# jyoung3131/oncilla

Hardware: AMD Instinct MI355X
Metric: remote put/get GiB/s + p50 ocm_alloc latency, 4 KiB-1 GiB, 1/2/4/8 MI355X (higher is better)
Workload: dtype uint8

## Files before the change

### csrc/include/ocm/xfer.h

```cpp
#pragma once
#include <hip/hip_runtime_api.h>

#include <cstdint>

#include "ocm/list.h"

namespace ocm {

struct XferArgs {
    char *lin;
    char *ext[kXferMaxExtents];
    uint64_t rem_off;
    uint64_t len;
    uint32_t unit_shift;
    uint32_t n_ext;
    uint32_t tile_shift;
    uint32_t put;
};

enum XferVariant : int {
    XFER_AUTO = 0,
    XFER_REG = 1,
    XFER_LDS = 2,
    XFER_DMA = 3,
    XFER_PCIE = 4,
    XFER_PUSH = 5,
};

struct XferTuning {
    int variant = XFER_AUTO;
    int max_blocks = 0;
    bool nontemporal = true;
    bool write_through = false;
};

struct XferDone {
    unsigned long long *flag = nullptr;
    unsigned int *cnt = nullptr;
    unsigned long long val = 0;
};

__host__ __device__ inline uint64_t xfer_first_tile(uint64_t rem_off, uint32_t tile_shift) {
    return rem_off & ~((1ull << tile_shift) - 1);
}
__host__ __device__ inline uint64_t xfer_tile_count(uint64_t rem_off, uint64_t len, uint32_t tile_shift) {
    const uint64_t mask = (1ull << tile_shift) - 1;
    return (((rem_off + len + mask) & ~mask) - (rem_off & ~mask)) >> tile_shift;
}

hipError_t xfer_normalize(XferArgs &a);

hipError_t xfer_launch(const XferArgs &a, const XferTuning &t, hipStream_t stream, const XferDone *done = nullptr);

hipError_t xfer_push_launch(const XferArgs &a, uint32_t ext_mask, int max_blocks, hipStream_t stream);

hipError_t xfer_copy(void *dst, const void *src, uint64_t bytes, const XferTuning &t, hipStream_t stream);

XferTuning xfer_tuning_from_env();

struct XferBatchOp {
    uint64_t lin_off;
    uint64_t rem_off;
    uint64_t len;
    uint64_t first_tile;
    uint32_t put;
    uint32_t pad;
};
static_assert(sizeof(XferBatchOp) == 40, "batch op layout");

constexpr int kXferInlineOps = 48;

struct XferBatchArgs : ListArgs<XferBatchOp, kXferInlineOps> {
    uint32_t abs_lin;
};
static_assert(list_args_fit<XferBatchArgs>, "kernarg segment limit");

inline uint64_t xfer_batch_plan(XferBatchOp *ops, uint32_t n, uint32_t tile_shift) {
    return list_plan(ops, n, [tile_shift](const XferBatchOp &op) {
        return op.len ? xfer_tile_count(op.rem_off, op.len, tile_shift) : 0;
    });
}
uint32_t xfer_batch_grid(uint64_t total_tiles, bool host_tier = false);
uint32_t xfer_batch_tile_shift(uint32_t n_ext, uint32_t unit_shift);
hipError_t xfer_batch_launch(const XferBatchArgs &a, const XferTuning &t, hipStream_t stream);
hipError_t xfer_batch_graph_node(hipGraph_t graph, hipGraphNode_t dep, const XferBatchArgs &a, const XferTuning &t,
// ... 119 lines not shown
```

### csrc/src/kernels/xfer.hip

```cpp
#include <hip/hip_runtime.h>

#include <cstring>

#include "ocm/xfer.h"
#include "xfer_copy.h"
#include "xfer_host.h"

namespace ocm {

namespace {

constexpr int kWaveSlice = (1 << kTileShift) / kWaves;
constexpr int kChunksPerWave = kWaveSlice / 1024;

template <class Cfg, bool MASKED = false>
__device__ __forceinline__ void copy_tiles(const XferArgs &a, uint32_t ext_mask = 0) {
    const uint64_t first = xfer_first_tile(a.rem_off, a.tile_shift);
    const uint64_t ntiles = xfer_tile_count(a.rem_off, a.len, a.tile_shift);
    const uint64_t r0 = a.rem_off;
    for (uint64_t ti = blockIdx.x; ti < ntiles; ti += gridDim.x) {
        if (MASKED && a.n_ext > 1) {
            const uint64_t lo = first + (ti << a.tile_shift);
            const uint64_t ts = lo > r0 ? lo : r0;
            const uint32_t e = (uint32_t)(ts >> a.unit_shift) % a.n_ext;
            if (!((ext_mask >> e) & 1u)) continue;
        }
        TileSpan s = tile_span(a, ti, first);
        copy_span<Cfg>(s.dst, s.src, s.n);
    }
}

template <int ST>
__global__ __launch_bounds__(kThreads) void xfer_reg_kernel(XferArgs a, XferDone d) {
    copy_tiles<BlockCopy<ST>>(a);
// ... 54 lines not shown
        }
        if (nt >= ntiles) break;
        ti = nt;
        cur = nxt;
        cur_staged = nxt_staged;
        slot ^= 1;
    }
}

template <bool NT>
__global__ __launch_bounds__(kThreads) void xfer_lds_kernel(XferArgs a, XferDone d) {
    __shared__ __attribute__((aligned(16))) char lds[2 * (1 << kTileShift)];
    const int wave = threadIdx.x >> 6, lane = threadIdx.x & 63;
    const uint64_t first = xfer_first_tile(a.rem_off, a.tile_shift);
    const uint64_t ntiles = xfer_tile_count(a.rem_off, a.len, a.tile_shift);
    uint64_t ti = blockIdx.x;
    if (ti < ntiles) lds_stream<NT>(a, lds, wave, lane, ti, first, ntiles);
    xfer_publish(d);
}

constexpr int kPcieUnroll = 2;
constexpr uint32_t kPcieTileShift = 13;
constexpr unsigned kPcieBlocksDefault = 128;

template <int SA>
using PcieCopy = CopyCfg<kThreads, kPcieUnroll, BufferAccess<kAuxNT, SA>>;

template <int SA>
__global__ __launch_bounds__(kThreads) void xfer_pcie_kernel(XferArgs a, XferDone d) {
    copy_tiles<PcieCopy<SA>>(a);
    xfer_publish(d);
}

__global__ __launch_bounds__(kThreads) void xfer_push_kernel(XferArgs a, uint32_t mask) {
    copy_tiles<BlockCopy<ST_NT>, true>(a, mask);
}

}

XferTuning xfer_tuning_from_env() {
    XferTuning t;
    const char *v = std::getenv("OCM_XFER_VARIANT");
    if (v && (!std::strcmp(v, "lds") || !std::strcmp(v, "2"))) t.variant = XFER_LDS;
    if (v && (!std::strcmp(v, "reg") || !std::strcmp(v, "1"))) t.variant = XFER_REG;
    if (v && (!std::strcmp(v, "pcie") || !std::strcmp(v, "4"))) t.variant = XFER_PCIE;
    if (v && (!std::strcmp(v, "push") || !std::strcmp(v, "5"))) t.variant = XFER_PUSH;
    t.max_blocks = kernels::env_int("OCM_XFER_BLOCKS", 0);
    t.nontemporal = kernels::env_int("OCM_XFER_NT", 1) != 0;
    t.write_through = kernels::env_int("OCM_XFER_NT", 1) == 2;
    return t;
}

hipError_t xfer_normalize(XferArgs &a) {
    if (a.n_ext < 1 || a.n_ext > (uint32_t)kXferMaxExtents) return hipErrorInvalidValue;
    a.tile_shift = kTileShift;
    if (a.n_ext > 1) {
        if (a.unit_shift < 4) return hipErrorInvalidValue;
        if (a.unit_shift < kTileShift) a.tile_shift = a.unit_shift;
    }
    return hipSuccess;
}

hipError_t xfer_launch(const XferArgs &in, const XferTuning &t, hipStream_t stream, const XferDone *done) {
    if (in.len == 0) return hipSuccess;
    XferArgs a = in;
    if (xfer_normalize(a) != hipSuccess) return hipErrorInvalidValue;
    const uint64_t ntiles = xfer_tile_count(a.rem_off, a.len, a.tile_shift);
    int variant = t.variant;
    if (variant == XFER_AUTO) variant = XFER_REG;
    const XferDone d0 = done ? *done : XferDone{};
    if (variant == XFER_PCIE) {
        if (a.tile_shift > kPcieTileShift) a.tile_shift = kPcieTileShift;
        const uint64_t tiles = xfer_tile_count(a.rem_off, a.len, a.tile_shift);
        const uint64_t cap = t.max_blocks > 0 ? (uint64_t)t.max_blocks : (uint64_t)kPcieBlocksDefault;
        const unsigned g = (unsigned)(tiles < cap ? tiles : cap);
        if (a.put && t.nontemporal)
            hipLaunchKernelGGL(xfer_pcie_kernel<kAuxSC1>, dim3(g), dim3(kThreads), 0, stream, a, d0);
        else
            hipLaunchKernelGGL(xfer_pcie_kernel<0>, dim3(g), dim3(kThreads), 0, stream, a, d0);
        return hipGetLastError();
    }
    if (a.tile_shift != kTileShift) variant = XFER_REG;
    int cap = t.max_blocks > 0 ? t.max_blocks : kernels::num_cus() * (variant == XFER_LDS ? 4 : 2);
    const unsigned grid = (unsigned)(ntiles < (uint64_t)cap ? ntiles : (uint64_t)cap);
    if (variant == XFER_LDS) {
        if (t.nontemporal)
            hipLaunchKernelGGL(xfer_lds_kernel<true>, dim3(grid), dim3(kThreads), 0, stream, a, d0);
        else
            hipLaunchKernelGGL(xfer_lds_kernel<false>, dim3(grid), dim3(kThreads), 0, stream, a, d0);
    } else {
        if (t.write_through)
            hipLaunchKernelGGL(xfer_reg_kernel<ST_WT>, dim3(grid), dim3(kThreads), 0, stream, a, d0);
        else if (t.nontemporal)
            hipLaunchKernelGGL(xfer_reg_kernel<ST_NT>, dim3(grid), dim3(kThreads), 0, stream, a, d0);
        else
            hipLaunchKernelGGL(xfer_reg_kernel<ST_PLAIN>, dim3(grid), dim3(kThreads), 0, stream, a, d0);
    }
    return hipGetLastError();
}

hipError_t xfer_push_launch(const XferArgs &in, uint32_t ext_mask, int max_blocks, hipStream_t stream) {
    if (in.len == 0 || ext_mask == 0) return hipSuccess;
    XferArgs a = in;
    if (a.put || xfer_normalize(a) != hipSuccess) return hipErrorInvalidValue;
    const uint64_t tiles = xfer_tile_count(a.rem_off, a.len, a.tile_shift);
    const uint32_t mine = (uint32_t)__builtin_popcount(ext_mask & ((1u << a.n_ext) - 1));
    const uint64_t own = a.n_ext > 1 ? (tiles * mine + a.n_ext - 1) / a.n_ext : tiles;
    const uint64_t cap = max_blocks > 0 ? (uint64_t)max_blocks : (uint64_t)kernels::num_cus() * 2;
    const unsigned g = (unsigned)(own < cap ? (own ? own : 1) : cap);
    hipLaunchKernelGGL(xfer_push_kernel, dim3(g), dim3(kThreads), 0, stream, a, ext_mask);
    return hipGetLastError();
}

hipError_t xfer_copy(void *dst, const void *src, uint64_t bytes, const XferTuning &t, hipStream_t stream) {
    XferArgs a;
// ... 12 lines not shown
```

### csrc/src/lib/config.cpp

```cpp
#include "config.h"

#include <algorithm>
#include <climits>
#include <cstdlib>
#include <cstring>

namespace ocmlib {

int env_int(const char *k, int dflt) {
    const char *v = std::getenv(k);
    return (v && *v) ? std::atoi(v) : dflt;
}

static uint64_t env_u64(const char *k, uint64_t dflt) {
    const char *v = std::getenv(k);
    return (v && *v) ? std::strtoull(v, nullptr, 0) : dflt;
}

static int env_clamped(const char *k, int dflt, int lo, int hi = INT_MAX) {
    return std::max(lo, std::min(env_int(k, dflt), hi));
}

static bool env_bool(const char *k, bool dflt) { return env_int(k, dflt ? 1 : 0) != 0; }

static uint64_t env_scaled(const char *k, uint64_t dflt, uint64_t per, int lo) {
    return per * (uint64_t)env_clamped(k, (int)(dflt / per), lo);
}

Config config_from_env() {
    Config c;
    c.rpc_timeout_ms = env_int("OCM_RPC_TIMEOUT_MS", c.rpc_timeout_ms);
    c.rpc_spin_ns = env_scaled("OCM_RPC_SPIN_US", c.rpc_spin_ns, 1000, 0);
    c.connect_timeout_ms = env_int("OCM_CONNECT_TIMEOUT_MS", c.connect_timeout_ms);
    c.shm_link = env_bool("OCM_SHM_LINK", c.shm_link);
    c.no_gpu = std::getenv("OCM_NO_GPU") != nullptr;
    c.net_streams = env_clamped("OCM_NET_STREAMS", c.net_streams, 1, 64);
    c.net_split_min = std::max<uint64_t>(4096, env_u64("OCM_NET_SPLIT_MIN", c.net_split_min));
    c.sync_mode = env_int("OCM_SYNC_MODE", c.sync_mode);
    c.n_lanes = env_int("OCM_ASYNC_LANES", c.n_lanes);
    c.pinned_keep = env_u64("OCM_PINNED_KEEP", c.pinned_keep);
    c.dev_cache_cap = env_u64("OCM_LOCAL_CACHE", c.dev_cache_cap);
    const char *he = std::getenv("OCM_HOST_ENGINE");
    c.host_engine_kernel = !(he && !std::strcmp(he, "sdma"));
    c.host_kernel_max = env_u64("OCM_HOST_KERNEL_MAX", c.host_engine_kernel ? c.host_kernel_max : 0);
    c.launch_flags = env_bool("OCM_LAUNCH_FLAG", c.launch_flags);
    c.launch_flag_max = env_u64("OCM_LAUNCH_FLAG_MAX", c.launch_flag_max);

    c.svc_eager = env_bool("OCM_SERVICE_EAGER", c.svc_eager);
    const char *sm = std::getenv("OCM_SERVICE_MAX");
    c.svc_max = env_u64("OCM_SERVICE_MAX", c.svc_max);
    c.svc_max_host = env_u64("OCM_SERVICE_MAX_HOST", sm && *sm ? c.svc_max : c.svc_max_host);
    c.svc_max_local = env_u64("OCM_SERVICE_MAX_LOCAL", c.svc_max_local);
    const char *q = std::getenv("OCM_SERVICE_QUEUE");
    c.svc_queue_aql = !(q && std::strcmp(q, "hip") == 0);
    c.svc_lanes_max = (unsigned)env_clamped("OCM_SERVICE_STREAMS", (int)c.svc_lanes_max, 1, 16);
    c.svc_blocks = (unsigned)env_clamped("OCM_SERVICE_BLOCKS", (int)c.svc_blocks, 1, 1024);
    c.svc_gang_host = (unsigned)env_clamped("OCM_SERVICE_GANG_HOST", (int)c.svc_gang_host, 1, 1024);
    c.svc_solo_tiles = (unsigned)env_clamped("OCM_SERVICE_SOLO_TILES", (int)c.svc_solo_tiles, 0);
    c.svc_solo_tiles_host_get = (unsigned)env_clamped("OCM_SERVICE_SOLO_TILES_HOST_GET", (int)c.svc_solo_tiles_host_get, 0);
    c.svc_proto = (unsigned)env_int("OCM_SERVICE_PROTO", (int)kServiceProtoDefault) & kServiceProtoMask;
    if (const int ps = env_int("OCM_SERVICE_POLL_SLEEP", -1); ps >= 0 && ps < 255)
        c.svc_proto |= (unsigned)(ps + 1) << kServicePollSleepShift;
    if (const int pj = env_int("OCM_SERVICE_POLL_JITTER", kServicePollJitterDefault); pj > 0 && pj < 16)
        c.svc_proto |= (unsigned)pj << kServicePollJitterShift;
    c.svc_force_strict = env_bool("OCM_SERVICE_STRICT", c.svc_force_strict);
    c.svc_direct = (unsigned)env_clamped("OCM_SERVICE_DIRECT", (int)c.svc_direct, 1, 1024);
    if (c.svc_direct > (unsigned)kServiceGangCopiesMax) c.svc_proto &= ~kServiceProtoCopies;
    c.svc_direct_max_host = env_u64("OCM_SERVICE_DIRECT_MAX_HOST", c.svc_direct_max_host);
    c.svc_direct_max_hbm = env_u64("OCM_SERVICE_DIRECT_MAX_HBM", c.svc_direct_max_hbm);
    c.svc_host_tile_shift_get = (unsigned)env_clamped("OCM_SERVICE_HOST_TILE_SHIFT_GET", (int)c.svc_host_tile_shift_get, 0);
    c.svc_host_tile_shift_put = (unsigned)env_clamped("OCM_SERVICE_HOST_TILE_SHIFT_PUT", (int)c.svc_host_tile_shift_put, 0);
    c.svc_host_tile_min = env_u64("OCM_SERVICE_HOST_TILE_MIN", c.svc_host_tile_min);
    c.svc_host_tile_max = env_u64("OCM_SERVICE_HOST_TILE_MAX", c.svc_host_tile_max);
    c.svc_host_get_narrow_min = env_u64("OCM_SERVICE_HOST_GET_NARROW_MIN", c.svc_host_get_narrow_min);
    c.svc_host_get_width = (unsigned)env_clamped("OCM_SERVICE_HOST_GET_WIDTH", (int)c.svc_host_get_width, 1, 1024);
    c.svc_park_kernel = env_bool("OCM_SERVICE_PARK_KERNEL", c.svc_park_kernel);
    c.svc_idle_ticks = env_scaled("OCM_SERVICE_IDLE_US", c.svc_idle_ticks, 100, 1);
    c.svc_degraded_idle_ticks = env_scaled("OCM_SERVICE_DEGRADED_IDLE_US", c.svc_degraded_idle_ticks, 100, 1);
    c.svc_lone_ticks = env_scaled("OCM_SERVICE_LONE_US", c.svc_lone_ticks, 100, 0);
// ... 18 lines not shown
```

### csrc/src/lib/config.h

```cpp
#pragma once
#include <cstdint>

#include "ocm/xfer.h"

struct lib_alloc;

namespace ocmlib {
using namespace ocm;
#pragma GCC visibility push(hidden)

constexpr uint64_t kServiceMaxDefault = 4ull << 20;
constexpr uint64_t kServiceMaxHostDefault = 16ull << 20;
constexpr int kServiceBlocksDefault = 128;
constexpr unsigned kServiceGangHostDefault = 32;
constexpr uint64_t kServiceMaxLocalDefault = 64ull << 20;
constexpr int kServiceSoloTilesDefault = 2;
constexpr int kServiceIdleUsDefault = 50;
constexpr int kServiceLoneUsDefault = 2000;
constexpr unsigned kServiceProtoDefault =
    kServiceProtoWT | kServiceProtoGangRec | kServiceProtoWCReq | kServiceProtoWgDone | kServiceProtoPipe;
constexpr int kServicePollJitterDefault = 3;
constexpr int kServiceDirectDefault = 16;
constexpr uint64_t kServiceDirectMaxHost = 4ull << 20;
constexpr uint64_t kServiceDirectMaxHbm = 1ull << 20;
constexpr uint64_t kLaunchFlagMaxDefault = 4ull << 20;

struct Config {
    int rpc_timeout_ms = 60000;
    uint64_t rpc_spin_ns = 50 * 1000;
    int connect_timeout_ms = 10000;
    bool shm_link = true;
    bool no_gpu = false;
    int net_streams = 4;
    uint64_t net_split_min = 1ull << 20;
    int sync_mode = 1;
    int n_lanes = 4;
    uint64_t pinned_keep = 2ull << 30;
    uint64_t dev_cache_cap = 1ull << 30;
    bool host_engine_kernel = true;
    uint64_t host_kernel_max = 0;
    bool launch_flags = true;
    uint64_t launch_flag_max = kLaunchFlagMaxDefault;

    bool svc_eager = true;
    uint64_t svc_max = kServiceMaxDefault;
    uint64_t svc_max_host = kServiceMaxHostDefault;
    uint64_t svc_max_local = kServiceMaxLocalDefault;
    uint64_t svc_limit(const lib_alloc *a) const;
    bool svc_queue_aql = true;
    unsigned svc_lanes_max = 4;
    unsigned svc_blocks = kServiceBlocksDefault;
    unsigned svc_gang_host = kServiceGangHostDefault;
    unsigned svc_solo_tiles = kServiceSoloTilesDefault;
    unsigned svc_solo_tiles_host_get = 1;
    unsigned svc_proto = kServiceProtoDefault | (unsigned)kServicePollJitterDefault << kServicePollJitterShift;
    bool svc_force_strict = false;
    unsigned svc_direct = kServiceDirectDefault;
    uint64_t svc_direct_max_host = kServiceDirectMaxHost;
    uint64_t svc_direct_max_hbm = kServiceDirectMaxHbm;
    unsigned svc_host_tile_shift_get = 14, svc_host_tile_shift_put = 14;
    uint64_t svc_host_tile_min = 64ull << 10;
    uint64_t svc_host_tile_max = 256ull << 10;
    uint64_t svc_host_get_narrow_min = 1ull << 20;
    unsigned svc_host_get_width = 12;
    bool svc_park_kernel = false;
    uint64_t svc_idle_ticks = 100ull * kServiceIdleUsDefault;
    uint64_t svc_degraded_idle_ticks = 100ull * 5000;
    uint64_t svc_lone_ticks = 100ull * kServiceLoneUsDefault;
    uint64_t svc_roster_wait_ns = 200 * 1000ull;
    uint64_t svc_timeout_ns = 10000 * 1000000ull;
    uint64_t svc_drain_ns = 10000 * 1000000ull;
    bool svc_box_reset_always = false;
    bool svc_relaunch_query = false;
    bool svc_prearm = false;
    uint64_t svc_arm_window_ns = 20 * 1000000ull;
// ... 14 lines not shown
```

### csrc/src/lib/introspect.cpp

```cpp
#include <cmath>

#include "internal.h"

using namespace ocm;
using namespace ocmlib;

extern "C" {


void ocm_x_counters(uint64_t out[28]) {
    const OpCounters &c = S().ctr;
    const uint64_t v[28] = {c.n_put,  c.n_get,    c.bytes_put, c.bytes_get,   c.n_alloc,     c.n_free,
                            c.n_copy, c.bytes_copy, c.ns_put,  c.ns_get,      c.ns_alloc,    c.ns_free,
                            c.n_batch, c.n_batch_ops, c.bytes_batch, c.ns_batch, c.n_batch_launches,
                            c.n_slab_fd, c.n_slab_path, c.n_link_rpc, c.n_link_wake,
                            c.n_quant, c.n_quant_ops, c.bytes_quant_src, c.bytes_quant_wire,
                            c.n_strided, c.n_strided_ops, c.bytes_strided};
    std::memcpy(out, v, sizeof(v));
}

void ocm_x_acc_counters(uint64_t out[3]) {
    const OpCounters &c = S().ctr;
    out[0] = c.n_acc;
    out[1] = c.n_acc_ops;
// ... 254 lines not shown
            }
        }
        rows++;
    }
    return rows;
}

void ocm_x_dump_stacks(const char *why) { dump_all_stacks(2, why ? why : "ocm_x_dump_stacks"); }

void ocm_x_set_slab_resolver(void *fn) {
    State &s = S();
    std::lock_guard<std::recursive_mutex> lk(s.mu);
    s.slab_resolver = reinterpret_cast<void *(*)(const unsigned char *)>(fn);
}

int ocm_x_service_pages(ocm_alloc_t a, uint64_t out[3]) {
    State &s = S();
    std::lock_guard<std::recursive_mutex> lk(s.mu);
    out[0] = reinterpret_cast<uint64_t>(s.svc_rec_pages);
    out[1] = reinterpret_cast<uint64_t>(s.svc);
    out[2] = (a && !a->ext.empty()) ? reinterpret_cast<uint64_t>(a->ext[0].hptr) : 0;
    return s.svc ? 0 : -1;
}

void ocm_x_set_tuning(int variant, int blocks, int nt) {
    State &s = S();
    std::lock_guard<std::recursive_mutex> lk(s.mu);
    s.tuning = tuning_of(variant, blocks, nt);
    s.dir_tuning[0] = s.dir_tuning[1] = XferTuning{};
}

int ocm_x_set_tuning_dir(int dir, int variant, int blocks, int nt) {
    if (dir != 0 && dir != 1) return -1;
    if (variant < XFER_AUTO || variant > XFER_PUSH || blocks < 0) return -1;
    State &s = S();
    std::lock_guard<std::recursive_mutex> lk(s.mu);
    s.dir_tuning[dir] = tuning_of(variant, blocks, nt);
    return 0;
}

int ocm_x_link_info(int dev, int peer, uint32_t *type, uint32_t *hops) {
    if (hipExtGetLinkTypeAndHopCount(dev, peer, type, hops) != hipSuccess) {
        (void)hipGetLastError();
        return -1;
    }
    return 0;
}

void ocm_x_layout(uint64_t out[8]) {
    out[0] = sizeof(Msg);
    out[1] = sizeof(struct ocm_params);
    out[2] = sizeof(struct ocm_alloc_params);
    out[3] = offsetof(Msg, u);
    out[4] = sizeof(Region);
    out[5] = sizeof(NodeConfig);
    out[6] = sizeof(AllocReq);
    out[7] = kHandleBytes;
}
}
```

### csrc/src/lib/transfer.cpp

```cpp
#include "internal.h"

namespace ocmlib {



void segments(const lib_alloc *a, uint64_t rem_off, uint64_t len, std::vector<Seg> &out) {
    out.clear();
    const int n = (int)a->ext.size();
    if (n == 1 || a->stripe_unit == 0) {
        out.push_back({0, rem_off, 0, len});
        return;
    }
    const uint64_t unit = a->stripe_unit;
    uint64_t pos = rem_off, done = 0;
    while (done < len) {
        const uint64_t u = pos / unit, within = pos % unit;
        const uint64_t take = std::min(unit - within, len - done);
        out.push_back({(int)(u % n), (u / n) * unit + within, done, take});
        pos += take;
        done += take;
    }
}


// ... 175 lines not shown
    segments(a, rem_off, len, segs);
    (void)copy_segs(a, segs.data(), segs.size(), put, lin, lloc, nullptr);
    return 0;
}

static int xfer_service(lib_alloc *a, bool put, char *lin, uint64_t rem_off, uint64_t len) {
    State &s = S();
    XferArgs x;
    if (pair_args(a, put, lin, rem_off, len, &x) != 0) return -2;
    if (wait_alloc(a) != 0) return -2;
    if (honor_dep(a, nullptr, true) != 0) return -2;
    const unsigned solo = (!put && !a->any_gpu) ? std::min(s.cfg.svc_solo_tiles, s.cfg.svc_solo_tiles_host_get)
                                                : s.cfg.svc_solo_tiles;
    return service_xfer(x, solo, a->any_gpu, a->any_peer || s.cfg.svc_force_strict);
}

static int xfer_push(lib_alloc *a, char *lin, uint64_t rem_off, uint64_t len, hipStream_t st, bool async) {
    before_launch();
    if (push_get(a, lin, rem_off, len, st, async) != 0) return -1;
    return async ? async_done(a, st) : 0;
}

static int xfer_kernel(lib_alloc *a, bool put, char *lin, uint64_t rem_off, uint64_t len, hipStream_t st, bool async,
                       XferDone *done) {
    State &s = S();
    if ((s.cfg.svc_park_kernel || !a->any_gpu) && len > s.cfg.svc_limit(a)) service_park();
    before_launch();
    XferArgs x;
    if (pair_args(a, put, lin, rem_off, len, &x) != 0) return -1;
    XferTuning t = dir_tuning(put);
    if (t.variant == XFER_AUTO) {
        bool same_gpu = true;
        for (auto &e : a->ext) same_gpu &= e.r.tier == TIER_GPU && e.r.owner_gpu == s.device;
        t.variant = !a->any_gpu ? XFER_PCIE : (same_gpu && len <= (256ull << 20)) ? XFER_LDS : XFER_REG;
    }
    XferDone dn;
    if (done && async && len <= s.cfg.launch_flag_max && s.cfg.launch_flags && s.lane_flags && st != s.stream &&
        a->lane >= 0 && a->ev) {
        dn.flag = s.lane_flags + (size_t)a->lane * 16;
        dn.cnt = s.lane_cnt + (size_t)a->lane * 32;
        dn.val = ++s.lane_flag_seq[(size_t)a->lane];
    }
    const hipError_t err = xfer_launch(x, t, st, dn.flag ? &dn : nullptr);
    if (err != hipSuccess) OCM_FAIL(-1, "transfer launch failed: %s", hipGetErrorString(err));
    if (done) *done = dn;
    return async ? async_done(a, st) : sync_stream();
}

static int xfer_dma(lib_alloc *a, bool put, char *lin, Loc lloc, uint64_t rem_off, uint64_t len, hipStream_t st,
                    bool async) {
    service_park();
    std::vector<Seg> segs;
    segments(a, rem_off, len, segs);
    bool cpu_piece = false;
    for (auto &g : segs) cpu_piece |= cpu_copies(lloc, a->ext[g.ext]);
    hipError_t err = hipSuccess;
    if (cpu_piece && (err = hipStreamSynchronize(st)) != hipSuccess)
        OCM_FAIL(-1, "ordering a host copy after queued work: %s", hipGetErrorString(err));
    err = copy_segs(a, segs.data(), segs.size(), put, lin, lloc, st);
    if (err != hipSuccess) OCM_FAIL(-1, "transfer launch failed: %s", hipGetErrorString(err));
    return async ? async_done(a, st) : sync_stream();
}

int xfer(lib_alloc *a, bool put, char *lin, Loc lloc, uint64_t rem_off, uint64_t len, bool async, XferDone *done) {
    State &s = S();
    if (done) *done = XferDone{};
    if (len == 0) return 0;
// ... 73 lines not shown
        for (size_t i = 0; i < a->ext.size(); i++) {
            x.ext[i] = nullptr;
            if (!((kv.second >> i) & 1u)) continue;
            x.ext[i] = extent_view(a->ext[i], d);
            if (!x.ext[i]) return -1;
        }
        DeviceGuard gd(d);
        hipError_t e = hipStreamWaitEvent(p->stream, s.push_order, 0);
        if (e == hipSuccess) e = xfer_push_launch(x, kv.second, s.dir_tuning[0].max_blocks, p->stream);
        if (e == hipSuccess) e = hipEventRecord(p->done, p->stream);
        if (e != hipSuccess) OCM_FAIL(-1, "push get on GPU %d: %s", d, hipGetErrorString(e));
        used.push_back(p);
        s.push_launches++;
    }
    for (PushDev *p : used) {
        const hipError_t e = async ? hipStreamWaitEvent(st, p->done, 0) : hipEventSynchronize(p->done);
        if (e != hipSuccess) OCM_FAIL(-1, "push get completion: %s", hipGetErrorString(e));
    }
    return 0;
}

int copy_local(void *dst, Loc dl, const void *src, Loc sl, size_t n) {
    State &s = S();
    if (n == 0) return 0;
    if (dl != LOC_DEVICE && sl != LOC_DEVICE) {
        std::memcpy(dst, src, n);
        return 0;
    }
    DeviceGuard g(s.device);
    hipError_t e;
    before_launch();
    if (dl == LOC_DEVICE && sl == LOC_DEVICE) {
        XferTuning t = s.tuning;
        if (t.variant == XFER_AUTO) t.variant = n <= (256ull << 20) ? XFER_LDS : XFER_REG;
        e = xfer_copy(dst, src, n, t, s.stream);
    } else
    {
        e = hipMemcpyAsync(dst, src, n, hipMemcpyDefault, s.stream);
    }
    if (e != hipSuccess) OCM_FAIL(-1, "local copy failed: %s", hipGetErrorString(e));
    return sync_stream();
}


}
```

### oncilla_amd/api.py

```python
from __future__ import annotations

import ctypes
import os
import threading
from typing import Optional

from .utils.paths import lib_path

OCM_LOCAL_HOST = 1
OCM_LOCAL_RMA = 2
OCM_REMOTE_RMA = 3
OCM_LOCAL_RDMA = 4
OCM_REMOTE_RDMA = 5
OCM_LOCAL_GPU = 6
OCM_REMOTE_GPU = 7

OCM_ALLOC_STRIPE = 1 << 0
OCM_ALLOC_HOST_TIER = 1 << 1
OCM_ALLOC_NO_SPILL = 1 << 2
OCM_ALLOC_ZERO = 1 << 3
OCM_ALLOC_LOOPBACK = 1 << 4

OCM_TIER_HOST = 1
OCM_TIER_GPU = 2
# ... 239 lines not shown
            "ocm_x_counters": (None, [ctypes.POINTER(u64)]),
            "ocm_x_acc_counters": (None, [ctypes.POINTER(u64)]),
            "ocm_x_quant_strided_counters": (None, [ctypes.POINTER(u64)]),
            "ocm_x_indexed_counters": (None, [ctypes.POINTER(u64)]),
            "ocm_x_service_stats": (None, [ctypes.POINTER(u64)]),
            "ocm_x_service_health": (None, [ctypes.POINTER(u64)]),
            "ocm_x_tick_stats": (ctypes.c_int, [ctypes.POINTER(u64)]),
            "ocm_x_place_stats": (ctypes.c_int, [ctypes.POINTER(u64)]),
            "ocm_x_quiesce": (None, []),
            "ocm_x_service_trace": (i32, [ctypes.POINTER(u64), i32]),
            "ocm_x_service_optrace": (i32, [ctypes.POINTER(u64), i32]),
            "ocm_x_set_slab_resolver": (None, [ctypes.c_void_p]),
            "ocm_x_dump_stacks": (None, [ctypes.c_char_p]),
            "ocm_x_service_cold": (None, [ctypes.POINTER(u64)]),
            "ocm_x_service_cold_reset": (None, []),
            "ocm_x_set_prearm": (i32, [i32]),
            "ocm_x_set_prearm_window": (i32, [i32]),
            "ocm_x_service_pages": (i32, [ctypes.c_void_p, ctypes.POINTER(u64)]),
            "ocm_x_adam": (i32, [vp, vp, vp, u64, u64, u64, ctypes.POINTER(ctypes.c_float), vp]),
            "ocm_x_adam_multi": (i32, [vp, i32, ctypes.POINTER(vp), ctypes.POINTER(vp), ctypes.POINTER(u64),
                                       ctypes.POINTER(u64), ctypes.POINTER(u64), ctypes.POINTER(u64),
                                       ctypes.POINTER(ctypes.c_float), i32, vp]),
            "ocm_x_adam_bf16": (i32, [vp, vp, vp, u64, u64, u64, u64, ctypes.POINTER(ctypes.c_float), vp]),
            "ocm_x_adam_multi_acc": (i32, [vp, vp, i32, ctypes.POINTER(vp), ctypes.POINTER(u64), ctypes.POINTER(u64),
                                           ctypes.POINTER(u64), ctypes.POINTER(u64), ctypes.POINTER(u64),
                                           ctypes.POINTER(ctypes.c_float), ctypes.c_float, ctypes.c_uint32, i32, vp]),
            "ocm_x_adam_rows": (i32, [vp, vp, ctypes.POINTER(OcmAdamRows), vp, vp, ctypes.POINTER(ctypes.c_float),
                                      ctypes.c_float, vp, vp]),
            "ocm_x_acc_sumsq": (i32, [vp, i32, ctypes.POINTER(u64), ctypes.POINTER(u64), vp, vp, vp, u64, vp]),
            "ocm_x_acc_sumsq_work_bytes": (u64, [i32]),
            "ocm_x_clip_scale": (ctypes.c_double, [ctypes.c_double, ctypes.c_double, ctypes.c_double]),
            "ocm_x_set_tuning": (None, [i32, i32, i32]),
            "ocm_x_set_tuning_dir": (i32, [i32, i32, i32, i32]),
            "ocm_x_batch": (i32, [i32, vp, ctypes.POINTER(vp), i32, u64, ctypes.POINTER(u64), i32, i32]),
            "ocm_x_link_info": (i32, [i32, i32, ctypes.POINTER(ctypes.c_uint32), ctypes.POINTER(ctypes.c_uint32)]),
            "ocm_x_extent_handle": (i32, [vp, i32, ctypes.c_char_p]),
            "ocm_x_extent_region": (i32, [vp, i32, ctypes.POINTER(u64)]),
            "ocm_x_xgmi_diag": (None, [ctypes.POINTER(u64)]),
            "ocm_x_link_layout": (None, [ctypes.POINTER(u64)]),
            "ocm_x_ipc_open": (i32, [i32, ctypes.c_char_p, ctypes.POINTER(vp)]),
            "ocm_x_ipc_close": (i32, [i32, vp]),
            "ocm_x_pattern_dev": (ctypes.c_longlong, [i32, vp, u64, u64, ctypes.c_uint32, i32]),
            "ocm_x_torch_pool_config": (None, [i32, ctypes.c_uint32]),
            "ocm_x_torch_pool_stats": (None, [ctypes.POINTER(u64)]),
        }
        for name, (res, args) in sigs.items():
            fn = getattr(lib, name)
            fn.restype = res
            fn.argtypes = args
        _lib = lib
        return lib


def _adam_hp(hp) -> tuple:
    hp = tuple(float(x) for x in hp)
    if len(hp) not in (6, 7):
        raise ValueError("Adam hyper-parameters: 6 values (Adam) or 7 (AdamW decay multiplier last)")
    if len(hp) == 6:
        hp += (float("nan"),)
    return hp + (1.0 - hp[0], 1.0 - hp[1])


def clip_scale(sumsq_total: float, scale: float, max_norm: float) -> float:
    return float(load().ocm_x_clip_scale(float(sumsq_total), float(scale), float(max_norm)))


# ... 245 lines not shown
            if dtype is not None or scale != 1.0:
                raise ValueError("acc_ops: an (n, 5) array carries each op's dtype and scale; pass neither beside it")
            rec["dt"][:n] = a[:, 3].astype(np.int64)
            with np.errstate(over="ignore"):
                rec["sc"][:n] = a[:, 4].astype(np.float32)
        else:
            if dtype is None:
                raise ValueError("acc_ops: an (n, 3) array needs a dtype")
            rec["dt"][:n] = acc_dtype(dtype)
            with np.errstate(over="ignore"):
                rec["sc"][:n] = np.float32(scale)
    b = BatchOps(rec.ctypes.data_as(ctypes.POINTER(OcmAccParams)), n)
    b.keep = rec
    b.acc = True
    return b


def acc_counters() -> dict:
    out = (ctypes.c_uint64 * len(ACC_COUNTER_KEYS))()
    load().ocm_x_acc_counters(out)
    return dict(zip(ACC_COUNTER_KEYS, [int(v) for v in out]))


def set_tuning(variant: int = 0, blocks: int = 0, nontemporal: bool = True) -> None:
    load().ocm_x_set_tuning(variant, blocks, 1 if nontemporal else 0)


def set_tuning_dir(op_flag: int, variant: int = 0, blocks: int = 0, nontemporal=True) -> None:
    nt = 2 if nontemporal == 2 else (1 if nontemporal else 0)
    if load().ocm_x_set_tuning_dir(op_flag, variant, blocks, nt) != 0:
        raise ValueError(f"bad tuning: op_flag={op_flag} variant={variant} blocks={blocks}")


def link_info(dev: int, peer: int) -> Optional[dict]:
    t, h = ctypes.c_uint32(), ctypes.c_uint32()
    if load().ocm_x_link_info(dev, peer, ctypes.byref(t), ctypes.byref(h)) != 0:
        return None
    return {"type": int(t.value), "hops": int(h.value)}


def counters() -> dict:
    out = (ctypes.c_uint64 * len(COUNTER_KEYS))()
    load().ocm_x_counters(out)
    return dict(zip(COUNTER_KEYS, [int(v) for v in out]))


def link_layout() -> dict:
    out = (ctypes.c_uint64 * 11)()
    load().ocm_x_link_layout(out)
    keys = ("bytes", "req_taken", "rsp_taken", "daemon_polling", "app_waiting", "req", "rsp", "slot", "seq", "slots",
            "magic")
    return dict(zip(keys, (int(x) for x in out)))


def xgmi_diag() -> dict:
    out = (ctypes.c_uint64 * 5)()
    load().ocm_x_xgmi_diag(out)
    return {"device": ctypes.c_int64(out[0]).value, "peer_access": int(out[1]), "ipc_imports": int(out[2]),
            "ipc_failures": int(out[3]), "push_launches": int(out[4])}


def quiesce() -> None:
    load().ocm_x_quiesce()


def service_stats() -> dict:
# ... 552 lines not shown
```

### oncilla_amd/models/workloads.py

```python
from __future__ import annotations

from typing import Iterable

from .. import api


def sweep_sizes(min_bytes: int = 4096, max_bytes: int = 1 << 30) -> list[int]:
    out, s = [], min_bytes
    while s <= max_bytes:
        out.append(s)
        s *= 2
    return out


def percentile(xs: list[float], q: float) -> float:
    ys = sorted(xs)
    if not ys:
        return float("nan")
    k = min(len(ys) - 1, max(0, int(round(q / 100.0 * (len(ys) - 1)))))
    return ys[k]


def alloc_latency(client: api.Client, kind: int, samples: int, local_bytes: int, remote_bytes: int = 0,
                  flags: int = 0, warmup: int = 5) -> dict:
# ... 59 lines not shown
            row[f"{key}_relaunches"] = rel
            row[f"{key}_n"] = len(xs)
            if rel and h0["relaunches"] < h1["relaunches"]:
                tot = lambda h: (h["relaunch_host_us_mean"] or 0) * h["relaunches"]
                row[f"{key}_relaunch_host_us"] = round((tot(h1) - tot(h0)) / (h1["relaunches"] - h0["relaunches"]), 2)
            dc = h1.get("cold_ops", 0) - h0.get("cold_ops", 0)
            if dc > 0:
                mean = lambda k: ((h1[k] or 0) * h1["cold_ops"] - (h0[k] or 0) * h0["cold_ops"]) / dc
                row[f"{key}_cold_split_us"] = {"dispatch_to_start": round(mean("cold_dispatch_to_start_us"), 2),
                                               "start_to_seen": round(mean("cold_start_to_seen_us"), 2),
                                               "total": round(mean("cold_total_us"), 2), "ops": dc}
        out[str(int(round(gap * 1e6)))] = row
    return out


def merge_idle_gap_rows(per_rank: list) -> dict:
    out = {}
    for gap in sorted({g for r in per_rank for g in r}, key=lambda g: int(g)):
        rows = [r[gap] for r in per_rank if gap in r]
        row = {}
        for k in sorted({k for x in rows for k in x}):
            vals = [x[k] for x in rows if x.get(k) is not None]
            if vals and isinstance(vals[0], dict):
                row[k] = {f: (sum if f == "ops" else max)([v[f] for v in vals if v.get(f) is not None])
                          for f in sorted({f for v in vals for f in v})}
                continue
            row[k] = (max(vals) if k.endswith("_us") else sum(vals)) if vals else None
        out[gap] = row
    return out


TUNING_CANDIDATES = {"auto": (0, 0, 1), "reg_b256": (1, 256, 1), "reg_b1024": (1, 1024, 1),
                     "reg_b2048": (1, 2048, 1), "reg_nt0": (1, 0, 0), "lds_default": (2, 0, 1),
                     "lds_b512": (2, 512, 1), "reg_wt": (1, 0, 2), "reg_wt_b1024": (1, 1024, 2), "dma": (3, 0, 1)}
PUSH_CANDIDATES = {"push": (5, 0, 1), "push_b1024": (5, 1024, 1)}
BASELINE_ONLY = frozenset({"dma"})
AUTOTUNE_MARGIN = 0.03


def default_candidates() -> dict:
    import os

    c = dict(TUNING_CANDIDATES)
    if os.environ.get("OCM_AUTOTUNE_PUSH") == "1":
        c.update(PUSH_CANDIDATES)
    return c


def _median(xs: list[float]) -> float:
    ys = sorted(xs)
    n = len(ys)
    return ys[n // 2] if n % 2 else 0.5 * (ys[n // 2 - 1] + ys[n // 2])


def autotune(alloc: api.Allocation, nbytes: int, reps: int = 5, gather=None, candidates: dict | None = None,
             margin: float = AUTOTUNE_MARGIN) -> dict:
    cands = dict(candidates or default_candidates())
    cands.setdefault("auto", (0, 0, 1))
    baselines = {n for n in cands if n in BASELINE_ONLY}
    gather = gather or (lambda obj: [obj])
    reps = max(1, reps)
    table = {}
    for name, (variant, blocks, nt) in cands.items():
        row = {}
        for op, key in ((0, "get"), (1, "put")):
            t, err = None, None
            try:
# ... 97 lines not shown
```

### oncilla_amd/ops/__init__.py

```python
from .acc import accumulate_reference
from .quant import (mx4_decode_reference, mx4_encode_reference, mx4_record_reference, mx4_rows_reference, mx8_decode_reference, mx8_encode_reference, mx8_record_reference, mx8_rows_reference)
from .xfer import XFER_AUTO, XFER_LDS, XFER_PCIE, XFER_PUSH, XFER_REG, batch, device_copy_seconds, striped_reference, xfer

__all__ = ["accumulate_reference", "XFER_AUTO", "XFER_LDS", "XFER_PCIE", "XFER_PUSH", "XFER_REG", "batch", "device_copy_seconds", "striped_reference", "xfer",
           "mx8_decode_reference", "mx8_encode_reference", "mx8_record_reference", "mx8_rows_reference",
           "mx4_decode_reference", "mx4_encode_reference", "mx4_record_reference", "mx4_rows_reference"]
```

### oncilla_amd/ops/xfer.py

```python
from __future__ import annotations

import ctypes

from .. import api

XFER_AUTO, XFER_REG, XFER_LDS, XFER_PCIE, XFER_PUSH = 0, 1, 2, 4, 5


def _ptr(t) -> int:
    return t.data_ptr()


def xfer(lin, exts: list, unit: int, rem_off: int, nbytes: int, put: bool, variant: int = XFER_AUTO,
         blocks: int = 0, sync: bool = True) -> None:
    lib = api.load()
    n = len(exts)
    arr = (ctypes.c_void_p * n)(*[_ptr(e) for e in exts])
    rc = lib.ocm_x_xfer(lin.device.index or 0, ctypes.c_void_p(_ptr(lin)), arr, n, unit, rem_off, nbytes,
                        1 if put else 0, variant, blocks, 1 if sync else 0)
    if rc != 0:
        raise api.OcmError("ocm_x_xfer failed")


def striped_reference(lin, exts: list, unit: int, rem_off: int, nbytes: int, put: bool) -> None:
    n = len(exts)
    pos, done = rem_off, 0
    while done < nbytes:
        u, within = divmod(pos, unit) if n > 1 else (0, pos)
        take = min((unit - within) if n > 1 else nbytes - done, nbytes - done)
        e = exts[u % n] if n > 1 else exts[0]
        eoff = (u // n) * unit + within if n > 1 else pos
        if put:
            e[eoff:eoff + take].copy_(lin[done:done + take])
        else:
            lin[done:done + take].copy_(e[eoff:eoff + take])
        pos += take
        done += take


# ... 18 lines not shown
```

Measured before the change: 52.94.

## Add streaming copy kernel with one tile per block for large same-GPU transfers

Adds an XFER_STREAM variant: a copy kernel with small 8 KiB tiles, low unroll, a high occupancy launch bound and one workgroup per tile, in place of a capped persistent grid. Auto selection now routes same-GPU transfers above a configurable LDS threshold (default 256 MiB) to this kernel instead of the register-copy kernel. The aim is more memory parallelism and latency hiding on very large local copies. It also adds per-variant launch counters (an atomic increment per launch) and tidies env parsing. The cost is millions of workgroups for GiB-sized copies and more scheduling overhead.

```diff
diff --git a/csrc/include/ocm/xfer.h b/csrc/include/ocm/xfer.h
--- a/csrc/include/ocm/xfer.h
+++ b/csrc/include/ocm/xfer.h
@@ -25,7 +25,20 @@
     XFER_DMA = 3,
     XFER_PCIE = 4,
     XFER_PUSH = 5,
-};
+    XFER_STREAM = 6,
+};
+
+inline int xfer_variant_from_name(const char *v) {
+    struct Name {
+        const char *name, *num;
+        int variant;
+    };
+    constexpr Name names[] = {{"reg", "1", XFER_REG},   {"lds", "2", XFER_LDS},      {"pcie", "4", XFER_PCIE},
+                              {"push", "5", XFER_PUSH}, {"stream", "6", XFER_STREAM}};
+    for (const Name &n : names)
+        if (v && (!__builtin_strcmp(v, n.name) || !__builtin_strcmp(v, n.num))) return n.variant;
+    return XFER_AUTO;
+}
 
 struct XferTuning {
     int variant = XFER_AUTO;
@@ -51,6 +64,8 @@
 hipError_t xfer_normalize(XferArgs &a);
 
 hipError_t xfer_launch(const XferArgs &a, const XferTuning &t, hipStream_t stream, const XferDone *done = nullptr);
+
+uint64_t xfer_launches(int variant);
 
 hipError_t xfer_push_launch(const XferArgs &a, uint32_t ext_mask, int max_blocks, hipStream_t stream);
 
diff --git a/csrc/src/kernels/xfer.hip b/csrc/src/kernels/xfer.hip
--- a/csrc/src/kernels/xfer.hip
+++ b/csrc/src/kernels/xfer.hip
@@ -1,5 +1,6 @@
 #include <hip/hip_runtime.h>
 
+#include <atomic>
 #include <cstring>
 
 #include "ocm/xfer.h"
@@ -120,19 +121,34 @@
     xfer_publish(d);
 }
 
+constexpr int kStreamUnroll = 2;
+constexpr uint32_t kStreamTileShift = 13;
+constexpr int kStreamWavesPerSimd = 8;
+
+template <bool NT>
+using StreamCopy = CopyCfg<kThreads, kStreamUnroll, BufferAccess<kAuxNT, NT ? kAuxNT : 0>>;
+
+template <bool NT>
+__global__ __launch_bounds__(kThreads, kStreamWavesPerSimd) void xfer_stream_kernel(XferArgs a, XferDone d) {
+    copy_tiles<StreamCopy<NT>>(a);
+    xfer_publish(d);
+}
+
 __global__ __launch_bounds__(kThreads) void xfer_push_kernel(XferArgs a, uint32_t mask) {
     copy_tiles<BlockCopy<ST_NT>, true>(a, mask);
 }
 
+std::atomic<uint64_t> g_launches[XFER_STREAM + 1];
+
+}
+
+uint64_t xfer_launches(int variant) {
+    return variant >= 0 && variant <= XFER_STREAM ? g_launches[variant].load(std::memory_order_relaxed) : 0;
 }
 
 XferTuning xfer_tuning_from_env() {
     XferTuning t;
-    const char *v = std::getenv("OCM_XFER_VARIANT");
-    if (v && (!std::strcmp(v, "lds") || !std::strcmp(v, "2"))) t.variant = XFER_LDS;
-    if (v && (!std::strcmp(v, "reg") || !std::strcmp(v, "1"))) t.variant = XFER_REG;
-    if (v && (!std::strcmp(v, "pcie") || !std::strcmp(v, "4"))) t.variant = XFER_PCIE;
-    if (v && (!std::strcmp(v, "push") || !std::strcmp(v, "5"))) t.variant = XFER_PUSH;
+    t.variant = xfer_variant_from_name(std::getenv("OCM_XFER_VARIANT"));
     t.max_blocks = kernels::env_int("OCM_XFER_BLOCKS", 0);
     t.nontemporal = kernels::env_int("OCM_XFER_NT", 1) != 0;
     t.write_through = kernels::env_int("OCM_XFER_NT", 1) == 2;
@@ -155,8 +171,10 @@
     if (xfer_normalize(a) != hipSuccess) return hipErrorInvalidValue;
     const uint64_t ntiles = xfer_tile_count(a.rem_off, a.len, a.tile_shift);
     int variant = t.variant;
-    if (variant == XFER_AUTO) variant = XFER_REG;
     const XferDone d0 = done ? *done : XferDone{};
+    if (variant != XFER_LDS && variant != XFER_PCIE && variant != XFER_STREAM) variant = XFER_REG;
+    if (a.tile_shift != kTileShift && variant == XFER_LDS) variant = XFER_REG;
+    g_launches[variant].fetch_add(1, std::memory_order_relaxed);
     if (variant == XFER_PCIE) {
         if (a.tile_shift > kPcieTileShift) a.tile_shift = kPcieTileShift;
         const uint64_t tiles = xfer_tile_count(a.rem_off, a.len, a.tile_shift);
@@ -168,7 +186,17 @@
             hipLaunchKernelGGL(xfer_pcie_kernel<0>, dim3(g), dim3(kThreads), 0, stream, a, d0);
         return hipGetLastError();
     }
-    if (a.tile_shift != kTileShift) variant = XFER_REG;
+    if (variant == XFER_STREAM) {
+        if (a.tile_shift > kStreamTileShift) a.tile_shift = kStreamTileShift;
+        const uint64_t tiles = xfer_tile_count(a.rem_off, a.len, a.tile_shift);
+        const uint64_t cap = t.max_blocks > 0 ? (uint64_t)t.max_blocks : (uint64_t)INT32_MAX;
+        const unsigned g = (unsigned)(tiles < cap ? tiles : cap);
+        if (t.nontemporal)
+            hipLaunchKernelGGL(xfer_stream_kernel<true>, dim3(g), dim3(kThreads), 0, stream, a, d0);
+        else
+            hipLaunchKernelGGL(xfer_stream_kernel<false>, dim3(g), dim3(kThreads), 0, stream, a, d0);
+        return hipGetLastError();
+    }
     int cap = t.max_blocks > 0 ? t.max_blocks : kernels::num_cus() * (variant == XFER_LDS ? 4 : 2);
     const unsigned grid = (unsigned)(ntiles < (uint64_t)cap ? ntiles : (uint64_t)cap);
     if (variant == XFER_LDS) {
diff --git a/csrc/src/lib/config.cpp b/csrc/src/lib/config.cpp
--- a/csrc/src/lib/config.cpp
+++ b/csrc/src/lib/config.cpp
@@ -45,6 +45,7 @@
     c.host_kernel_max = env_u64("OCM_HOST_KERNEL_MAX", c.host_engine_kernel ? c.host_kernel_max : 0);
     c.launch_flags = env_bool("OCM_LAUNCH_FLAG", c.launch_flags);
     c.launch_flag_max = env_u64("OCM_LAUNCH_FLAG_MAX", c.launch_flag_max);
+    c.xfer_lds_max = env_u64("OCM_XFER_LDS_MAX", c.xfer_lds_max);
 
     c.svc_eager = env_bool("OCM_SERVICE_EAGER", c.svc_eager);
     const char *sm = std::getenv("OCM_SERVICE_MAX");
diff --git a/csrc/src/lib/config.h b/csrc/src/lib/config.h
--- a/csrc/src/lib/config.h
+++ b/csrc/src/lib/config.h
@@ -24,6 +24,7 @@
 constexpr uint64_t kServiceDirectMaxHost = 4ull << 20;
 constexpr uint64_t kServiceDirectMaxHbm = 1ull << 20;
 constexpr uint64_t kLaunchFlagMaxDefault = 4ull << 20;
+constexpr uint64_t kXferLdsMaxDefault = 256ull << 20;
 
 struct Config {
     int rpc_timeout_ms = 60000;
@@ -41,6 +42,8 @@
     uint64_t host_kernel_max = 0;
     bool launch_flags = true;
     uint64_t launch_flag_max = kLaunchFlagMaxDefault;
+    uint64_t xfer_lds_max = kXferLdsMaxDefault;
+    int xfer_local_variant(uint64_t len) const { return len <= xfer_lds_max ? XFER_LDS : XFER_STREAM; }
 
     bool svc_eager = true;
     uint64_t svc_max = kServiceMaxDefault;
diff --git a/csrc/src/lib/introspect.cpp b/csrc/src/lib/introspect.cpp
--- a/csrc/src/lib/introspect.cpp
+++ b/csrc/src/lib/introspect.cpp
@@ -310,12 +310,14 @@
 
 int ocm_x_set_tuning_dir(int dir, int variant, int blocks, int nt) {
     if (dir != 0 && dir != 1) return -1;
-    if (variant < XFER_AUTO || variant > XFER_PUSH || blocks < 0) return -1;
+    if (variant < XFER_AUTO || variant > XFER_STREAM || blocks < 0) return -1;
     State &s = S();
     std::lock_guard<std::recursive_mutex> lk(s.mu);
     s.dir_tuning[dir] = tuning_of(variant, blocks, nt);
     return 0;
 }
+
+uint64_t ocm_x_xfer_launches(int variant) { return xfer_launches(variant); }
 
 int ocm_x_link_info(int dev, int peer, uint32_t *type, uint32_t *hops) {
     if (hipExtGetLinkTypeAndHopCount(dev, peer, type, hops) != hipSuccess) {
diff --git a/csrc/src/lib/transfer.cpp b/csrc/src/lib/transfer.cpp
--- a/csrc/src/lib/transfer.cpp
+++ b/csrc/src/lib/transfer.cpp
@@ -231,7 +231,7 @@
     if (t.variant == XFER_AUTO) {
         bool same_gpu = true;
         for (auto &e : a->ext) same_gpu &= e.r.tier == TIER_GPU && e.r.owner_gpu == s.device;
-        t.variant = !a->any_gpu ? XFER_PCIE : (same_gpu && len <= (256ull << 20)) ? XFER_LDS : XFER_REG;
+        t.variant = !a->any_gpu ? XFER_PCIE : same_gpu ? s.cfg.xfer_local_variant(len) : XFER_REG;
     }
     XferDone dn;
     if (done && async && len <= s.cfg.launch_flag_max && s.cfg.launch_flags && s.lane_flags && st != s.stream &&
@@ -371,7 +371,7 @@
     before_launch();
     if (dl == LOC_DEVICE && sl == LOC_DEVICE) {
         XferTuning t = s.tuning;
-        if (t.variant == XFER_AUTO) t.variant = n <= (256ull << 20) ? XFER_LDS : XFER_REG;
+        if (t.variant == XFER_AUTO) t.variant = s.cfg.xfer_local_variant(n);
         e = xfer_copy(dst, src, n, t, s.stream);
     } else
     {
diff --git a/oncilla_amd/api.py b/oncilla_amd/api.py
--- a/oncilla_amd/api.py
+++ b/oncilla_amd/api.py
@@ -295,6 +295,7 @@
             "ocm_x_clip_scale": (ctypes.c_double, [ctypes.c_double, ctypes.c_double, ctypes.c_double]),
             "ocm_x_set_tuning": (None, [i32, i32, i32]),
             "ocm_x_set_tuning_dir": (i32, [i32, i32, i32, i32]),
+            "ocm_x_xfer_launches": (u64, [i32]),
             "ocm_x_batch": (i32, [i32, vp, ctypes.POINTER(vp), i32, u64, ctypes.POINTER(u64), i32, i32]),
             "ocm_x_link_info": (i32, [i32, i32, ctypes.POINTER(ctypes.c_uint32), ctypes.POINTER(ctypes.c_uint32)]),
             "ocm_x_extent_handle": (i32, [vp, i32, ctypes.c_char_p]),
@@ -606,6 +607,10 @@
         raise ValueError(f"bad tuning: op_flag={op_flag} variant={variant} blocks={blocks}")
 
 
+def xfer_launches(variant: int) -> int:
+    return int(load().ocm_x_xfer_launches(variant))
+
+
 def link_info(dev: int, peer: int) -> Optional[dict]:
     t, h = ctypes.c_uint32(), ctypes.c_uint32()
     if load().ocm_x_link_info(dev, peer, ctypes.byref(t), ctypes.byref(h)) != 0:
diff --git a/oncilla_amd/models/workloads.py b/oncilla_amd/models/workloads.py
--- a/oncilla_amd/models/workloads.py
+++ b/oncilla_amd/models/workloads.py
@@ -115,7 +115,8 @@
 
 TUNING_CANDIDATES = {"auto": (0, 0, 1), "reg_b256": (1, 256, 1), "reg_b1024": (1, 1024, 1),
                      "reg_b2048": (1, 2048, 1), "reg_nt0": (1, 0, 0), "lds_default": (2, 0, 1),
-                     "lds_b512": (2, 512, 1), "reg_wt": (1, 0, 2), "reg_wt_b1024": (1, 1024, 2), "dma": (3, 0, 1)}
+                     "lds_b512": (2, 512, 1), "reg_wt": (1, 0, 2), "reg_wt_b1024": (1, 1024, 2), "stream": (6, 0, 1),
+                     "dma": (3, 0, 1)}
 PUSH_CANDIDATES = {"push": (5, 0, 1), "push_b1024": (5, 1024, 1)}
 BASELINE_ONLY = frozenset({"dma"})
 AUTOTUNE_MARGIN = 0.03
diff --git a/oncilla_amd/ops/__init__.py b/oncilla_amd/ops/__init__.py
--- a/oncilla_amd/ops/__init__.py
+++ b/oncilla_amd/ops/__init__.py
@@ -1,7 +1,7 @@
 from .acc import accumulate_reference
 from .quant import (mx4_decode_reference, mx4_encode_reference, mx4_record_reference, mx4_rows_reference, mx8_decode_reference, mx8_encode_reference, mx8_record_reference, mx8_rows_reference)
-from .xfer import XFER_AUTO, XFER_LDS, XFER_PCIE, XFER_PUSH, XFER_REG, batch, device_copy_seconds, striped_reference, xfer
+from .xfer import XFER_AUTO, XFER_LDS, XFER_PCIE, XFER_PUSH, XFER_REG, XFER_STREAM, batch, device_copy_seconds, striped_reference, xfer
 
-__all__ = ["accumulate_reference", "XFER_AUTO", "XFER_LDS", "XFER_PCIE", "XFER_PUSH", "XFER_REG", "batch", "device_copy_seconds", "striped_reference", "xfer",
+__all__ = ["accumulate_reference", "XFER_AUTO", "XFER_LDS", "XFER_PCIE", "XFER_PUSH", "XFER_REG", "XFER_STREAM", "batch", "device_copy_seconds", "striped_reference", "xfer",
            "mx8_decode_reference", "mx8_encode_reference", "mx8_record_reference", "mx8_rows_reference",
            "mx4_decode_reference", "mx4_encode_reference", "mx4_record_reference", "mx4_rows_reference"]
diff --git a/oncilla_amd/ops/xfer.py b/oncilla_amd/ops/xfer.py
--- a/oncilla_amd/ops/xfer.py
+++ b/oncilla_amd/ops/xfer.py
@@ -4,7 +4,7 @@
 
 from .. import api
 
-XFER_AUTO, XFER_REG, XFER_LDS, XFER_PCIE, XFER_PUSH = 0, 1, 2, 4, 5
+XFER_AUTO, XFER_REG, XFER_LDS, XFER_PCIE, XFER_PUSH, XFER_STREAM = 0, 1, 2, 4, 5, 6
 
 
 def _ptr(t) -> int:
```

New measurement: 53.00, median of 6. About the same (+0.1%).
